# strawberrylady99/mythril

Measured on AMD Instinct MI355X. Metric: candidate assignments evaluated/sec (node) + time-to-first-model vs z3, higher is better.
Workload: dtype u32

## Files before the change

mythril_amd/csrc/jit_asm.cpp:

```cpp
#include <algorithm>
#include <array>
#include <cstdio>
#include <cstring>
#include <functional>
#include <map>
#include <set>
#include <sstream>
#include <string>
#include <vector>

#include "jit.hpp"

namespace mg {

namespace {

struct AsmFail {
  std::string why;
};
[[noreturn]] void fail(const std::string& w) { throw AsmFail{w}; }

inline uint32_t Lw(uint32_t w) { return (w + 31) / 32; }
inline uint32_t topmask(uint32_t w) { return (w & 31) ? ((1u << (w & 31)) - 1u) : 0xFFFFFFFFu; }
inline uint32_t gsalt(uint32_t c, uint32_t j) { return c * 0x9E3779B9u + j * 0x85EBCA6Bu + 0x27D4EB2Fu; }
// ... 241 lines not shown
    std::vector<int32_t> dix(P.vwidth.size(), -1);
    for (size_t k = 0; k < v.size(); k++)
      if (v[k].dst != MG_NONE && v[k].dst < dix.size() && dix[v[k].dst] < 0) dix[v[k].dst] = (int32_t)k;
    std::map<uint32_t, int32_t> coord_at;
    for (size_t k = 0; k < v.size(); k++)
      if (v[k].op == K_COORD && !coord_at.count(v[k].p0)) coord_at[v[k].p0] = (int32_t)k;
    auto operands = [&](const Instr& in, std::vector<int32_t>& out) {
      out.clear();
      auto add = [&](uint32_t id) {
        if (id != MG_NONE && id < dix.size() && dix[id] >= 0) out.push_back(dix[id]);
      };
      switch (in.op) {
        case K_CONST: break;
        case K_COORD:
          if (!eval_kernel && in.p0 < specs.size()) {
            const GenSpec& sp = specs[in.p0];
            if ((sp.kind & 0xFFu) == MG_GEN_MIXED && sp.p[3] != MG_NONE && (sp.p[2] & 0xFFFFu)) {
              auto it = coord_at.find(sp.p[3]);
              if (it != coord_at.end()) out.push_back(it->second);
            }
          }
          break;
        case K_LOOKUP:
          add(in.a);
          add(in.p0);
          for (uint32_t q = 0; q < 2 * in.c; q++) add(P.vaux[in.p1 + q]);
          break;
        case K_NOT: case K_NEG: case K_EXTRACT: case K_ZEXT: case K_SEXT: case K_ASSERT: case K_COPY: case K_WATCH:
          add(in.a);
          break;
        case K_ITE:
          add(in.a);
          add(in.b);
          add(in.c);
          break;
        default:
          add(in.a);
          add(in.b);
          break;
      }
    };
    std::vector<char> done(v.size(), 0);
    std::vector<Instr> out;
    out.reserve(v.size());
    std::vector<int32_t> ops;
    auto visit = [&](int32_t root) {
      std::vector<std::pair<int32_t, size_t>> st{{root, 0}};
      std::vector<std::vector<int32_t>> opl;
      opl.emplace_back();
      operands(v[root], opl.back());
      while (!st.empty()) {
        auto& top = st.back();
        if (done[top.first]) {
          st.pop_back();
          opl.pop_back();
          continue;
        }
        if (top.second < opl.back().size()) {
          const int32_t o = opl.back()[top.second++];
          if (!done[o]) {
            st.push_back({o, 0});
            opl.emplace_back();
            operands(v[o], opl.back());
          }
          continue;
        }
        done[top.first] = 1;
        out.push_back(v[top.first]);
        st.pop_back();
        opl.pop_back();
      }
    };
    if (eval_kernel && greedy_on()) {
      greedy_roots(v, operands, done, visit);
    } else if (!eval_kernel && heavy_last_on()) {
      heavy_last_roots(v, operands, done, visit);
    } else {
      for (size_t k = 0; k < v.size(); k++)
        if (v[k].op == K_ASSERT || v[k].op == K_WATCH) visit((int32_t)k);
    }
    for (size_t k = 0; k < v.size(); k++)
      if (!done[k]) visit((int32_t)k);
    code.swap(out);
  }
  static bool heavy_last_on() {
    static const bool on = [] {
      const char* g = getenv("MYTHGPU_JIT_ASM_HEAVY_LAST");
      return !(g && g[0] == '0');
    }();
    return on;
  }
  uint32_t op_weight(const Instr& in) const {
    const uint32_t w = (in.dst != MG_NONE && in.dst < P.vwidth.size()) ? P.vwidth[in.dst] : 32u;
    const uint32_t L = std::max(1u, Lw(std::max(w, in.op >= K_EQ && in.op <= K_UMUL_NOOVF ? in.p1 : w)));
    switch (in.op) {
      case K_KECCAK: return 2500u * (in.p0 / 136u + 1u);
      case K_EXP: return 1500u;
      case K_UDIV: case K_UREM: case K_SDIV: case K_SREM: case K_SMOD: return 600u;
      case K_MUL: return 4u * L * L;
      case K_UMUL_NOOVF: return 8u * L * L;
      case K_SHL: case K_LSHR: case K_ASHR: return 4u * L;
      case K_LOOKUP: return 2u * Lw(in.b) * std::max(1u, in.c);
      case K_COORD: return 8u * L;
      default: return L;
    }
  }
  static bool heavy_op(uint32_t op) {
    return op == K_KECCAK || op == K_EXP || op == K_UDIV || op == K_UREM || op == K_SDIV || op == K_SREM || op == K_SMOD;
  }
  template <class Ops, class Visit>
  void heavy_last_roots(const std::vector<Instr>& v, Ops& operands, const std::vector<char>& done, Visit& visit) {
    std::vector<int32_t> roots;
    for (size_t k = 0; k < v.size(); k++)
      if (v[k].op == K_ASSERT) roots.push_back((int32_t)k);
    std::vector<int32_t> mark(v.size(), -1), st, ops;
    int32_t stamp = 0;
    auto cone_cost = [&](int32_t r, bool& heavy) -> uint64_t {
      uint64_t c = 0;
      heavy = false;
      st.assign(1, r);
      mark[r] = ++stamp;
      while (!st.empty()) {
        const int32_t x = st.back();
        st.pop_back();
        c += op_weight(v[x]);
        heavy = heavy || heavy_op(v[x].op);
        operands(v[x], ops);
        for (int32_t o : ops)
          if (!done[o] && mark[o] != stamp) {
            mark[o] = stamp;
            st.push_back(o);
          }
      }
      return c;
    };
    std::vector<char> taken(roots.size(), 0);
    for (size_t step = 0; step < roots.size(); step++) {
      size_t pick = roots.size();
      uint64_t best = UINT64_MAX;
      for (size_t i = 0; i < roots.size(); i++) {
        if (taken[i]) continue;
        bool heavy = false;
        const uint64_t c = cone_cost(roots[i], heavy);
        if (!heavy) {
          pick = i;
          break;
        }
        if (c < best) {
          best = c;
          pick = i;
        }
      }
      taken[pick] = 1;
      visit(roots[pick]);
    }
  }
  static bool greedy_on() {
    static const bool on = [] {
      const char* g = getenv("MYTHGPU_JIT_ASM_GREEDY");
      return g && g[0] == '1';
    }();
    return on;
  }
  template <class Ops, class Visit>
  void greedy_roots(const std::vector<Instr>& v, Ops& operands, const std::vector<char>& done, Visit& visit) {
    const size_t n = v.size();
// ... 1108 lines not shown
    auto r = hby.equal_range(g);
    std::vector<std::vector<uint64_t>> keys;
    for (auto it = r.first; it != r.second; ++it) keys.push_back(it->second);
    hby.erase(r.first, r.second);
    for (const auto& k : keys) {
      auto it = hcache.find(k);
      if (it == hcache.end()) continue;
      const Limb d = it->second;
      hcache.erase(it);
      h_last.erase(k);
      drop(d);
    }
  }

  std::map<std::pair<uint32_t, uint32_t>, Limb> eqdiff;

  struct MEnt {
    Mask m;
    uint32_t tag = 0;
    uint64_t used = 0;
  };
  typedef std::vector<uint64_t> MKey;
  std::map<MKey, MEnt> mcache;
  uint32_t mc_hits = 0, mc_evictions = 0, mc_spills = 0;
  static bool no_mask_cache() {
    static const bool off = [] {
      const char* g = getenv("MYTHGPU_JIT_ASM_NO_MASK_CACHE");
      return g && g[0] == '1';
    }();
    return off;
  }
  bool mcache_on() const { return lvn_on && caches && !cond && !no_mask_cache(); }
  bool mcache_get(const MKey& key, Mask& m) {
    if (key.empty() || !mcache_on()) return false;
    auto it = mcache.find(key);
    if (it == mcache.end()) return false;
    E.scheck(it->second.m.s, it->second.tag);
    it->second.used = ++tick;
    m = it->second.m;
    E.sretain(m);
    mc_hits++;
    return true;
  }
  void mcache_put(const MKey& key, const Mask& m) {
    if (key.empty() || m.k != 2 || !mcache_on() || mcache.count(key)) return;
    MEnt e;
    e.m = m;
    e.tag = E.sgen[m.s];
    e.used = ++tick;
    E.sretain(m);
    mcache[key] = e;
  }
  bool mcache_evict() {
    auto best = mcache.end();
    for (auto it = mcache.begin(); it != mcache.end(); ++it)
      if (best == mcache.end() || it->second.used < best->second.used) best = it;
    if (best == mcache.end()) return false;
    E.srelease(best->second.m);
    mcache.erase(best);
    mc_evictions++;
    return true;
  }
  template <class F>
  void mcache_drop_if(F&& f) {
    for (auto it = mcache.begin(); it != mcache.end();) {
      if (f(it->first)) {
        E.srelease(it->second.m);
        it = mcache.erase(it);
      } else {
        ++it;
      }
    }
  }
  void mcache_forget(uint32_t id) {
    if (mcache.empty()) return;
    mcache_drop_if([&](const MKey& k) { return k[0] == 0 && (k[1] == id || k[2] == id); });
  }
  void mcache_free(uint32_t g) {
    if (mcache.empty()) return;
    mcache_drop_if([&](const MKey& k) { return (k[0] == 1 && k[1] == g) || (k[0] == 2 && (k[1] == g || k[3] == g)); });
  }
  void mcache_note() {
    E.o << "  ; mask cache: " << mc_hits << " hits, " << mc_evictions << " evictions, " << mc_spills << " mask spills\n";
  }
  int mcache_spare() const {
    int n = 0;
    for (const auto& kv : mcache) n += E.sref[kv.second.m.s] == 1;
    return n;
  }
  MKey idx_key(uint64_t kind, const Limb& idx) const {
    if (!idx.reg() || !idx.g || (int)idx.v < E.vfirst || E.vgen[idx.v] != idx.g) return {};
    return MKey{kind, idx.g, idx.v};
  }

  Mask eq_ids(uint32_t a, uint32_t b, uint32_t Lk) {
    PinScope pin_(*this, {a, b});
    const auto key = std::minmax(a, b);
    const MKey mkey{0, key.first, key.second};
    {
      Mask hit;
      if (mcache_get(mkey, hit)) {
        if (eqdiff.count(key)) eq_last[key] = ++tick;
        return hit;
      }
    }
    auto it = eqdiff.find(key);
    if (it != eqdiff.end()) {
      eq_last[key] = ++tick;
      Mask m;
      m.k = 2;
      m.s = E.salloc();
      E.valu("v_cmp_eq_u32_e64 " + SP(m.s) + ", 0, " + VL(it->second), {}, {m.s, m.s + 1});
      mcache_put(mkey, m);
      return m;
    }
    std::vector<std::pair<Limb, Limb>> prs;
    for (uint32_t j = 0; j < Lk; j++) prs.push_back({limb(a, j), limb(b, j)});
    Limb keep{};
    const Mask m = eq_mask(prs, &keep);
    if (keep.reg() && caches) {
      eqdiff[key] = keep;
      eq_last[key] = ++tick;
    }
    else if (keep.reg()) drop(keep);
    mcache_put(mkey, m);
    return m;
  }
  template <class M, class T>
  static typename M::iterator lru(M& m, T& last) {
    auto best = m.end();
    uint64_t bt = ~0ull;
    for (auto it = m.begin(); it != m.end(); ++it) {
      auto l = last.find(it->first);
      const uint64_t t = l == last.end() ? 0 : l->second;
      if (t < bt) {
        bt = t;
        best = it;
      }
    }
    return best;
  }
  bool evict_one() {
    if (!litcache.empty()) {
      auto it = lru(litcache, lit_last);
      const Limb d = it->second;
      lit_last.erase(it->first);
      litcache.erase(it);
      drop(d);
      return true;
    }
    if (!xcache.empty()) {
      auto it = lru(xcache, x_last);
      const Limb d = it->second;
      x_last.erase(it->first);
      xcache.erase(it);
      drop(d);
      return true;
    }
    if (!hcache.empty()) {
      auto it = lru(hcache, h_last);
      const Limb d = it->second;
      h_last.erase(it->first);
      hcache.erase(it);
      drop(d);
      return true;
    }
    if (!eqdiff.empty()) {
      auto it = lru(eqdiff, eq_last);
      const Limb d = it->second;
      eq_last.erase(it->first);
      eqdiff.erase(it);
      drop(d);
      return true;
    }
    return false;
  }
  size_t cur_k = 0;
  void note(const char* phase) {
    static const bool annotate = getenv("MYTHGPU_JIT_ASM_ANNOTATE") != nullptr;
    if (annotate) E.o << "  ; vcode " << cur_k << " " << phase << "\n";
  }
  bool spill_mask() {
    if (cond || cur_k >= code.size()) return false;
    const Instr& in = code[cur_k];
    auto operand = [&](uint32_t id) {
      if (id == in.a || id == in.b || id == in.c) return true;
      if (in.op == K_LOOKUP) {
        if (id == in.p0) return true;
        for (uint32_t q = 0; q < 2 * in.c; q++)
          if (P.vaux[in.p1 + q] == id) return true;
      }
      return false;
    };
    int64_t best = -1;
    int32_t bl = -1;
    for (uint32_t id = 0; id < val.size(); id++) {
      const Val& x = val[id];
      if (!x.def || x.m.k != 2 || E.sref[x.m.s] != 1 || operand(id)) continue;
      const int32_t lu = id < last.size() ? last[id] : -1;
      if (lu > bl) {
        bl = lu;
        best = id;
      }
// ... 1228 lines not shown
    if (!spill_on || cond) return false;
    int best = -1;
    int32_t bl = -1;
    for (uint32_t id = 0; id < val.size(); id++) {
      const Val& x = val[id];
      if (!x.def || is_spilled(id) || is_view(id) || P.vwidth[id] <= 32) continue;
      if (std::find(pinned.begin(), pinned.end(), id) != pinned.end()) continue;
      int regs = 0;
      bool own = true;
      for (const Limb& l : x.l)
        if (l.reg()) {
          regs++;
          own = own && (int)l.v >= E.vfirst && E.vref[l.v] == 1;
        }
      if (regs < 2 || !own) continue;
      const int32_t lu = id < last.size() ? last[id] : -1;
      if (lu > bl) {
        bl = lu;
        best = (int)id;
      }
    }
    if (best < 0) return false;
    Val& x = val[best];
    std::vector<int> at(x.l.size(), -1);
    for (size_t j = 0; j < x.l.size(); j++) {
      if (!x.l[j].reg()) continue;
      uint32_t sl = 0;
      while (sl < slot_busy.size() && slot_busy[sl]) sl++;
      if ((sl | 1u) > spill_cap()) fail("out of VGPRs (spill slots)");
      if (sl == slot_busy.size()) slot_busy.push_back(0);
      slot_busy[sl] = 1;
      spill_hwm = std::max(spill_hwm, sl + 1);
      E.mem("ds_write_b32 " + VL(spill_v) + ", " + VL(x.l[j]) + " offset:" + std::to_string(sl * 4u));
      at[j] = (int)sl;
    }
    E.ctl("s_waitcnt lgkmcnt(0)");
    for (size_t j = 0; j < x.l.size(); j++)
      if (at[j] >= 0) {
        drop(x.l[j]);
        x.l[j] = Limb{};
      }
    spill_at[best] = at;
    spills++;
    return true;
  }
  uint32_t spills = 0;
  void reload(uint32_t id) {
    if (cond) fail("a spilled value read under a branch");
    if (std::find(pinned.begin(), pinned.end(), id) == pinned.end())
      fail("internal: a spilled value read where it is not pinned");
    Val& x = val[id];
    const std::vector<int> at = spill_at[id];
    spill_at[id].clear();
    for (size_t j = 0; j < at.size(); j++) {
      if (at[j] < 0) continue;
      const Limb d = fresh();
      E.mem("ds_read_b32 " + VL(d) + ", " + VL(spill_v) + " offset:" + std::to_string((uint32_t)at[j] * 4u));
      x.l[j] = d;
    }
    E.ctl("s_waitcnt lgkmcnt(0)");
    for (int sl : at)
      if (sl >= 0) slot_busy[sl] = 0;
  }

  void kill(uint32_t id) {
    Val& x = val[id];
    if (is_spilled(id)) {
      for (int sl : spill_at[id])
        if (sl >= 0) slot_busy[sl] = 0;
      spill_at[id].clear();
    }
    for (auto& l : x.l) drop(l);
    x.l.clear();
    E.srelease(x.m);
    x.m = Mask{};
  }
  std::vector<Limb> limbs(uint32_t id, uint32_t n) {
    std::vector<Limb> r(n);
    for (uint32_t j = 0; j < n; j++) r[j] = limb(id, j);
    return r;
  }
  uint32_t demanded(uint32_t d) const { return need[d] ? 64 - (uint32_t)__builtin_clzll(need[d]) : 0; }

  bool lit_divisor(uint32_t b, uint32_t Ld) const {
    const Instr* bd = def_of(b);
    bool ok = bd && bd->op == K_CONST;
    for (uint32_t j = 1; ok && j < Ld; j++) ok = P.consts[bd->p0 + j] == 0;
    return ok;
  }
  void drop_all(std::vector<Limb>& v) {
    for (auto& x : v) drop(x);
    v.clear();
  }
  std::vector<Limb> own(const std::vector<Limb>& x, uint32_t n) {
    std::vector<Limb> r(n);
    for (uint32_t j = 0; j < n; j++) {
      const Limb s = j < x.size() && x[j].k != LU ? x[j] : Lit(0);
      r[j] = fresh();
      E.valu("v_mov_b32_e32 " + VL(r[j]) + ", " + src(s));
    }
    return r;
  }
  int sreg() { return E.salloc(); }
  void sfree(int s) {
    Mask m;
    m.k = 2;
    m.s = s;
    E.srelease(m);
  }
  Mask mask_new() {
    Mask m;
    m.k = 2;
    m.s = E.salloc();
    return m;
  }
  void vsel(const Limb& d, const Limb& f, const Limb& t, const Mask& m) {
    E.valu("v_cndmask_b32_e64 " + VL(d) + ", " + VL(f) + ", " + VL(t) + ", " + SP(m.s), {m.s, m.s + 1});
  }
  Mask vcmp(const char* op, const Limb& a, uint32_t k) {
    Mask m = mask_new();
    if (inl(k)) {
      E.valu(std::string("v_cmp_") + op + "_u32_e64 " + SP(m.s) + ", " + VL(a) + ", " + imm(k), {}, {m.s, m.s + 1});
    } else {
      E.salu("s_mov_b32 s41, " + hexs(k), {41});
      E.valu(std::string("v_cmp_") + op + "_u32_e64 " + SP(m.s) + ", " + VL(a) + ", s41", {41}, {m.s, m.s + 1});
    }
    return m;
  }

  Limb bitlen(const std::vector<Limb>& x) {
    const Limb bl = fresh();
    E.valu("v_mov_b32_e32 " + VL(bl) + ", 0");
    for (uint32_t j = 0; j < x.size(); j++) {
      const Limb l = x[j];
      if (l.k == LU || (l.lit() && l.v == 0)) continue;
      if (l.lit()) {
        E.valu("v_mov_b32_e32 " + VL(bl) + ", " + imm(32 * j + 32 - (uint32_t)__builtin_clz(l.v)));
        continue;
      }
      const Limb t = fresh();
      E.valu("v_ffbh_u32_e32 " + VL(t) + ", " + VL(l));
      E.valu("v_sub_u32_e32 " + VL(t) + ", " + imm(32 * j + 32) + ", " + VL(t));
      const Mask nz = vcmp("ne", l, 0);
      vsel(bl, bl, t, nz);
      E.srelease(nz);
      drop(t);
    }
    return bl;
  }
  void wave_max(const Limb& v, uint32_t bits, int s) {
    const int c = sreg();
    const Mask m = mask_new();
    E.salu("s_mov_b32 " + S(s) + ", 0", {s});
    for (int b = (int)bits - 1; b >= 0; b--) {
      E.salu("s_add_u32 " + S(c) + ", " + S(s) + ", " + imm(1u << b), {c});
      E.valu("v_cmp_ge_u32_e64 " + SP(m.s) + ", " + VL(v) + ", " + S(c), {c}, {m.s, m.s + 1});
      E.salu("s_cmp_lg_u64 " + SP(m.s) + ", 0");
      E.salu("s_cselect_b32 " + S(s) + ", " + S(c) + ", " + S(s), {s});
    }
    E.srelease(m);
    sfree(c);
  }

  void limb_barrel(std::vector<Limb>& x, const Limb& s, bool left, const Limb& fill) {
    const uint32_t Lx = (uint32_t)x.size();
    const Limb q = fresh();
// ... 1075 lines not shown
            r[j] = Lit(in.op == K_AND ? (a.v & b.v) : in.op == K_OR ? (a.v | b.v) : (a.v ^ b.v));
            continue;
          }
          const Limb l = a.lit() ? a : b, v = a.lit() ? b : a;
          if (l.lit()) {
            if ((in.op == K_AND && l.v == 0xFFFFFFFFu) || (in.op != K_AND && l.v == 0)) {
              E.retain(v);
              r[j] = v;
              continue;
            }
            if (in.op == K_AND && l.v == 0) { r[j] = Lit(0); continue; }
            if (in.op == K_OR && l.v == 0xFFFFFFFFu) { r[j] = Lit(0xFFFFFFFFu); continue; }
          }
          if (in.op != K_XOR && a == b) {
            E.retain(a);
            r[j] = a;
            continue;
          }
          const char* op = in.op == K_AND ? "v_and_b32_e32 " : in.op == K_OR ? "v_or_b32_e32 " : "v_xor_b32_e32 ";
          const Limb dd = fresh();
          E.valu(op + VL(dd) + ", " + src(l.lit() ? l : a) + ", " + VL(l.lit() ? v : b));
          r[j] = dd;
        }
        set(d, r);
        break;
      }
      case K_NOT: {
        if (W == 1) {
          set_mask(d, mnot(mask_of(in.a)));
          break;
        }
        std::vector<Limb> r(Ld);
        for (uint32_t j = 0; j < Ld; j++) {
          if (!(need[d] >> j & 1)) continue;
          const Limb a = limb(in.a, j);
          if (a.lit()) {
            r[j] = Lit(~a.v);
            continue;
          }
          const Limb dd = fresh();
          E.valu("v_not_b32_e32 " + VL(dd) + ", " + VL(a));
          r[j] = dd;
        }
        mask_top(r, W);
        set(d, r);
        break;
      }
      case K_COPY: {
        if (W == 1 && val[in.a].m.k) {
          E.sretain(val[in.a].m);
          val[d].m = val[in.a].m;
        }
        if (is_spilled(in.a)) reload(in.a);
        std::vector<Limb> r = val[in.a].l;
        for (auto& x : r) E.retain(x);
        set(d, r);
        break;
      }
      case K_ITE: {
        const Mask c = mask_of(in.a);
        if (W == 1) {
          if (c.k == 1) {
            const Mask x = mask_of(c.ones ? in.b : in.c);
            E.sretain(x);
            set_mask(d, x);
            break;
          }
          const Mask t = mop("and", c, mask_of(in.b));
          const Mask e = mask_of(in.c);
          Mask f;
          if (e.k == 1) {
            if (e.ones) {
              f = mnot(c);
            } else {
              f.k = 1;
              f.ones = false;
            }
          } else {
            f = mop_andn(e, c);
          }
          set_mask(d, mop("or", t, f));
          E.srelease(t);
          E.srelease(f);
          break;
        }
        std::vector<Limb> r(Ld);
        if (c.k == 1) {
          for (uint32_t j = 0; j < Ld; j++) {
            if (!(need[d] >> j & 1)) continue;
            r[j] = limb(c.ones ? in.b : in.c, j);
            E.retain(r[j]);
          }
          set(d, r);
          break;
        }
        if (c.k == 2 && !no_ite_e64() && !E.fresh_valu_write(c.s)) {
          for (uint32_t j = 0; j < Ld; j++) {
            if (!(need[d] >> j & 1)) continue;
            r[j] = sel_mask(limb(in.b, j), limb(in.c, j), c);
          }
          set(d, r);
          break;
        }
        mask_to_vcc(c);
        for (uint32_t j = 0; j < Ld; j++) {
          if (!(need[d] >> j & 1)) continue;
          r[j] = sel(limb(in.b, j), limb(in.c, j));
        }
        set(d, r);
        break;
      }
      case K_EQ: {
        const uint32_t La = Lw(in.p1);
        if (in.p1 == 1) {
          set_mask(d, mnot_xor(mask_of(in.a), mask_of(in.b)));
          break;
        }
        set_mask(d, no_eq_cache() ? [&] {
          std::vector<std::pair<Limb, Limb>> prs;
          for (uint32_t j = 0; j < La; j++) prs.push_back({limb(in.a, j), limb(in.b, j)});
          return eq_mask(prs);
        }() : eq_ids(in.a, in.b, La));
        break;
      }
      case K_ULT: case K_ULE: case K_SLT: case K_SLE: {
        const uint32_t La = Lw(in.p1);
        const bool sgn = in.op == K_SLT || in.op == K_SLE;
        if (in.p1 == 1) {
          const Mask a = mask_of(in.a), b = mask_of(in.b);
          Mask lt = sgn ? mop_andn(a, b) : mop_andn(b, a);
          if (in.op == K_ULE || in.op == K_SLE) {
            const Mask gt = sgn ? mop_andn(b, a) : mop_andn(a, b);
            const Mask le = mnot(gt);
            E.srelease(gt);
            E.srelease(lt);
            lt = le;
          }
          set_mask(d, lt);
          break;
        }
        slt_many = sgn && ((in.a < slt_lits.size() && slt_lits[in.a] >= 3) || (in.b < slt_lits.size() && slt_lits[in.b] >= 3));
        if (in.op == K_ULT || in.op == K_SLT) {
          set_mask(d, lt_mask(limbs(in.a, La), limbs(in.b, La), in.p1, sgn));
        } else {
          const Mask gt = lt_mask(limbs(in.b, La), limbs(in.a, La), in.p1, sgn);
          set_mask(d, mnot(gt));
          E.srelease(gt);
        }
        break;
      }
      case K_CONCAT: case K_EXTRACT: {
        std::vector<Limb> r(Ld);
        for (uint32_t j = 0; j < Ld; j++)
          if (need[d] >> j & 1) r[j] = field_of(in, 32 * j, std::min(32u, W - 32 * j));
        set(d, r);
        break;
      }
      case K_ZEXT: {
        const uint32_t La = Lw(in.p1);
        std::vector<Limb> r(Ld, Lit(0));
        for (uint32_t j = 0; j < La && j < Ld; j++) {
          if (!(need[d] >> j & 1)) continue;
          r[j] = limb(in.a, j);
          E.retain(r[j]);
        }
        set(d, r);
// ... 7 lines not shown
          r[j] = limb(in.a, j);
          E.retain(r[j]);
        }
        const Limb t = limb(in.a, La - 1);
        Limb top, f;
        if (t.lit()) {
          const uint32_t s = (wa - 1) & 31;
          const int32_t x = (int32_t)(t.v << (31 - s)) >> (31 - s);
          top = Lit((uint32_t)x);
          f = Lit(x < 0 ? 0xFFFFFFFFu : 0u);
        } else {
          if (wa & 31) {
            top = fresh();
            E.valu("v_bfe_i32 " + VL(top) + ", " + VL(t) + ", 0, " + std::to_string(wa & 31));
          } else {
            top = t;
            E.retain(top);
          }
          f = fresh();
          E.valu("v_ashrrev_i32_e32 " + VL(f) + ", 31, " + VL(top));
        }
        r[La - 1] = top;
        for (uint32_t j = La; j < Ld; j++) {
          r[j] = f;
          E.retain(f);
        }
        drop(f);
        mask_top(r, W);
        set(d, r);
        break;
      }
      case K_LOOKUP: {
        const uint32_t Lk = Lw(in.b), n = in.c;
        auto key_test = [&](uint32_t kv) -> Mask {
          if (!no_eq_cache()) return eq_ids(in.a, kv, Lk);
          std::vector<std::pair<Limb, Limb>> prs;
          for (uint32_t j = 0; j < Lk; j++) prs.push_back({limb(in.a, j), limb(kv, j)});
          return eq_mask(prs);
        };
        if (in.wd == 1 && !no_bool_lookup()) {
          Mask cur = mask_of(in.p0);
          E.sretain(cur);
          for (int32_t p = (int32_t)n - 1; p >= 0; p--) {
            const uint32_t kv = P.vaux[in.p1 + 2 * p], vv = P.vaux[in.p1 + 2 * p + 1];
            const Mask h = key_test(kv);
            if (h.k == 1) {
              if (h.ones) {
                E.srelease(cur);
                cur = mask_of(vv);
                E.sretain(cur);
              }
              continue;
            }
            const Mask vm = mask_of(vv);
            Mask nc;
            if (cur.k == 1 && !cur.ones) {
              nc = mop("and", h, vm);
            } else if (cur.k == 1 && vm.k == 2) {
              nc.k = 2;
              nc.s = E.salloc();
              E.salu("s_orn2_b64 " + SP(nc.s) + ", " + SP(vm.s) + ", " + SP(h.s), {nc.s, nc.s + 1});
            } else if (cur.k == 1) {
              if (vm.ones) {
                nc.k = 1;
                nc.ones = true;
              } else {
                nc = mnot(h);
              }
            } else if (vm.k == 1) {
              nc = vm.ones ? mop("or", h, cur) : mop_andn(cur, h);
            } else {
              const Mask t = mop("and", h, vm);
              const Mask f = mop_andn(cur, h);
              nc = mop("or", t, f);
              E.srelease(t);
              E.srelease(f);
            }
            E.srelease(cur);
            E.srelease(h);
            cur = nc;
          }
          set_mask(d, cur);
          break;
        }
        if (n >= 2 && n <= 5 && !no_lookup_runs() && E.sfree() + mcache_spare() >= (int)(n + n * (n - 1) / 2 + 4)) {
          std::vector<Mask> hs;
          std::vector<uint32_t> ps;
          int base = -1;
          for (int32_t p = (int32_t)n - 1; p >= 0; p--) {
            const Mask h = key_test(P.vaux[in.p1 + 2 * p]);
            if (h.k == 1) {
              if (h.ones) {
                for (auto& m : hs) E.srelease(m);
                hs.clear();
                ps.clear();
                base = p;
              }
              continue;
            }
            hs.push_back(h);
            ps.push_back((uint32_t)p);
          }
          const uint32_t dflt = base >= 0 ? P.vaux[in.p1 + 2 * base + 1] : in.p0;
          std::map<std::pair<size_t, size_t>, Mask> ors;
          auto run_mask = [&](size_t a, size_t b) -> Mask {
            if (a == b) return hs[a];
            auto it = ors.find({a, b});
            if (it != ors.end()) return it->second;
            const Mask prev = b - 1 == a ? hs[a] : ors.at({a, b - 1});
            const Mask m = mop("or", prev, hs[b]);
            ors[{a, b}] = m;
            return m;
          };
          std::vector<Limb> res(Ld);
          for (uint32_t j = 0; j < Ld; j++) {
            if (!(need[d] >> j & 1)) continue;
            Limb c = limb(dflt, j);
            E.retain(c);
            for (size_t a = 0; a < ps.size();) {
              const Limb v = limb(P.vaux[in.p1 + 2 * ps[a] + 1], j);
              size_t b = a;
              while (b + 1 < ps.size() && limb(P.vaux[in.p1 + 2 * ps[b + 1] + 1], j) == v) b++;
              if (!(v == c)) {
                for (size_t q = a + 1; q < b; q++) run_mask(a, q);
                const Mask m = run_mask(a, b);
                const Limb t = v3(v), f = v3(c);
                const Limb r = fresh();
                E.valu("v_cndmask_b32_e64 " + VL(r) + ", " + src(f) + ", " + src(t) + ", " + SP(m.s), {m.s, m.s + 1});
                drop(t);
                drop(f);
                drop(c);
                c = r;
              }
              a = b + 1;
            }
            res[j] = c;
          }
          for (auto& kv : ors) E.srelease(kv.second);
          for (auto& m : hs) E.srelease(m);
          set(d, res);
          break;
        }
        std::vector<Limb> cur(Ld);
        for (uint32_t j = 0; j < Ld; j++) {
          if (!(need[d] >> j & 1)) continue;
          cur[j] = limb(in.p0, j);
          E.retain(cur[j]);
        }
        for (int32_t p = (int32_t)n - 1; p >= 0; p--) {
          const uint32_t kv = P.vaux[in.p1 + 2 * p], vv = P.vaux[in.p1 + 2 * p + 1];
          Mask h;
          if (no_eq_cache()) {
            std::vector<std::pair<Limb, Limb>> prs;
            for (uint32_t j = 0; j < Lk; j++) prs.push_back({limb(in.a, j), limb(kv, j)});
            h = eq_mask(prs);
          } else {
            h = eq_ids(in.a, kv, Lk);
          }
          if (h.k == 1) {
            if (h.ones) {
              for (uint32_t j = 0; j < Ld; j++) {
                if (!(need[d] >> j & 1)) continue;
                drop(cur[j]);
                cur[j] = limb(vv, j);
                E.retain(cur[j]);
              }
// ... 92 lines not shown
    }();
    return on;
  }
  static bool no_bool_lookup() {
    static const bool on = [] {
      const char* g = getenv("MYTHGPU_JIT_ASM_NO_BOOL_LOOKUP");
      return g && g[0] == '1';
    }();
    return on;
  }
  static bool no_eq_cache() {
    static const bool on = [] {
      const char* g = getenv("MYTHGPU_JIT_ASM_NO_EQ_CACHE");
      return g && g[0] == '1';
    }();
    return on;
  }
  static bool gen_only() {
    static const bool on = [] {
      const char* g = getenv("MYTHGPU_JIT_ASM_GEN_ONLY");
      return g && g[0] == '1';
    }();
    return on;
  }
  static bool debug_live() {
    static const bool on = getenv("MYTHGPU_JIT_ASM_DEBUG") != nullptr;
    return on;
  }
  void operands_of(const Instr& in, size_t k, std::vector<uint32_t>& out) {
    std::function<void(uint32_t)> add = [&](uint32_t id) {
      if (id == MG_NONE || id >= val.size()) return;
      out.push_back(id);
      if (is_view(id)) {
        const Instr& vi = code[def[id]];
        add(vi.a);
        if (vi.op == K_CONCAT) add(vi.b);
      }
    };
    switch (in.op) {
      case K_CONST: break;
      case K_COORD: if (copysrc[k] != MG_NONE) add(copysrc[k]); break;
      case K_LOOKUP:
        add(in.a);
        add(in.p0);
        for (uint32_t q = 0; q < in.c; q++) add(P.vaux[in.p1 + 2 * q + 1]);
        break;
      default:
        add(in.a);
        if (in.op != K_NOT && in.op != K_NEG && in.op != K_EXTRACT && in.op != K_ZEXT && in.op != K_SEXT &&
            in.op != K_ASSERT && in.op != K_COPY && in.op != K_WATCH)
          add(in.b);
        if (in.op == K_ITE) add(in.c);
        break;
    }
  }
  void body(const std::string& next) {
    eqdiff.clear();
    mcache.clear();
    mc_hits = mc_evictions = mc_spills = 0;
    mulshare.clear();
    xcache.clear();
    xby.clear();
    hcache.clear();
    hby.clear();
    h_last.clear();
    litcache.clear();
    lit_last.clear();
    x_last.clear();
    eq_last.clear();
    dlimb.clear();
    E.on_free = [this](uint32_t g) {
      xcache_free(g);
      hcache_free(g);
      dlimb_free(g);
      mcache_free(g);
    };
    E.on_pressure = [this]() { return evict_one(); };
    E.on_hard = [this]() { return spill_one(); };
    spill_at.assign(val.size(), {});
    slot_busy.clear();
    pinned.clear();
    E.on_spressure = [this]() { return mcache_evict() || spill_mask(); };
    lvn_on = true;
    static const bool annotate = getenv("MYTHGPU_JIT_ASM_ANNOTATE") != nullptr;
    for (size_t k = 0; k < code.size(); k++) {
      const Instr& in = code[k];
      cur_k = k;
      if (is_view(in.dst)) continue;
      if (annotate)
        E.o << "  ; vcode " << k << " op " << in.op << " w " << in.wd << " dst " << in.dst << " a " << in.a << " b " << in.b
            << "\n";
      if (spill_on) {
        pinned.clear();
        operands_of(in, k, pinned);
        for (size_t q = 0; q < pinned.size(); q++)
          if (is_spilled(pinned[q])) reload(pinned[q]);
      }
      emit(in, k, next);
      if (spill_on) pinned.clear();
      if (debug_live()) {
        int used = 0;
        for (int r = E.vfirst; r < 256; r++) used += E.vref[r] > 0;
        fprintf(stderr, "asm live %zu op %u w %u: %d VGPRs\n", k, in.op, in.wd, used);
        static const long at = getenv("MYTHGPU_JIT_ASM_DEBUG_AT") ? atol(getenv("MYTHGPU_JIT_ASM_DEBUG_AT")) : -1;
        if ((long)k == at) {
          std::map<uint32_t, int> byop;
          for (uint32_t id = 0; id < val.size(); id++) {
            if (!val[id].def) continue;
            int regs = 0;
            for (const auto& l : val[id].l) regs += l.reg();
            if (regs && def[id] >= 0) byop[code[def[id]].op] += regs;
          }
          for (const auto& kv : byop) fprintf(stderr, "  live from op %u: %d limbs\n", kv.first, kv.second);
        }
      }
      auto done = [&](uint32_t id) {
        if (id != MG_NONE && id < last.size() && last[id] <= (int32_t)k && val[id].def) {
          kill(id);
          val[id].def = false;
          if (!eqdiff.empty()) eq_forget(id);
          mcache_forget(id);
        }
      };
      if (in.dst != MG_NONE && in.dst < last.size() && last[in.dst] < 0) done(in.dst);
      switch (in.op) {
        case K_CONST: break;
        case K_WATCH:
          if (eval_kernel) done(in.a);
          break;
        case K_COORD:
          if (copysrc[k] != MG_NONE) done(copysrc[k]);
          break;
        case K_LOOKUP:
          done(in.a);
          done(in.p0);
          for (uint32_t q = 0; q < 2 * in.c; q++) done(P.vaux[in.p1 + q]);
          break;
        default:
          done(in.a);
          if (in.b != MG_NONE) done(in.b);
          if (in.op == K_ITE) done(in.c);
          if (in.op == K_CONCAT || in.op == K_EXTRACT) {
            std::function<void(uint32_t)> through = [&](uint32_t id) {
              if (!is_view(id)) return;
              const Instr& vi = code[def[id]];
              done(vi.a);
              through(vi.a);
              if (vi.op == K_CONCAT) {
                done(vi.b);
                through(vi.b);
              }
            };
            through(in.a);
            if (in.op == K_CONCAT) through(in.b);
          }
          break;
      }
    }
    for (auto& kv : mulshare)
      for (auto& t : kv.second) drop(t);
    mulshare.clear();
    for (auto& kv : eqdiff) drop(kv.second);
    eqdiff.clear();
    mcache_drop_if([](const MKey&) { return true; });
    xcache_clear();
    litcache_clear();
    lvn_on = false;
    E.on_free = nullptr;
    E.on_pressure = nullptr;
    E.on_hard = nullptr;
// ... 711 lines not shown
      << "    .amdhsa_user_sgpr_count 2\n    .amdhsa_user_sgpr_kernarg_segment_ptr 1\n"
      << "    .amdhsa_system_sgpr_workgroup_id_x 1\n    .amdhsa_system_vgpr_workitem_id 0\n"
      << "    .amdhsa_next_free_vgpr " << nv << "\n    .amdhsa_next_free_sgpr " << ns << "\n"
      << "    .amdhsa_accum_offset " << accum << "\n    .amdhsa_reserve_vcc 1\n"
      << "    .amdhsa_float_denorm_mode_32 3\n    .amdhsa_float_denorm_mode_16_64 3\n"
      << "  .end_amdhsa_kernel\n  .text\n";
    labels = E.nlab;
    meta_lds = lds_words * 4;
    meta_vgpr[name] = nv;
    meta_sgpr[name] = ns + 6;
    return o.str();
  }
  std::map<std::string, int> meta_vgpr, meta_sgpr;
  uint32_t meta_lds = 0;
};

std::string metadata(const std::map<std::string, int>& vg, const std::map<std::string, int>& sg, bool with_gen,
                     uint32_t lds_bytes) {
  std::ostringstream o;
  auto arg = [&](uint32_t off, uint32_t size, const char* kind, bool global) {
    o << "      - .offset: " << off << "\n        .size: " << size << "\n        .value_kind: " << kind << "\n";
    if (global) o << "        .address_space: global\n";
  };
  o << "  .amdgpu_metadata\n---\namdhsa.kernels:\n";
  for (const char* name : {"mgj_search", "mgj_gen"}) {
    const bool gen = std::strcmp(name, "mgj_gen") == 0;
    if (gen && !with_gen) continue;
    o << "  - .args:\n";
    arg(0, 8, "global_buffer", true);
    for (uint32_t k = 0; k < 4; k++) arg(8 + 8 * k, 8, "by_value", false);
    arg(40, 8, "global_buffer", true);
    if (gen) {
      arg(48, 4, "by_value", false);
    } else {
      arg(48, 4, "by_value", false);
      arg(52, 4, "by_value", false);
    }
    o << "    .group_segment_fixed_size: " << lds_bytes << "\n    .kernarg_segment_align: 8\n"
      << "    .kernarg_segment_size: " << (gen ? 52 : 56) << "\n    .max_flat_workgroup_size: 256\n"
      << "    .name: " << name << "\n    .private_segment_fixed_size: 0\n"
      << "    .sgpr_count: " << sg.at(name) << "\n    .sgpr_spill_count: 0\n"
      << "    .symbol: " << name << ".kd\n    .uniform_work_group_size: 1\n    .uses_dynamic_stack: false\n"
      << "    .vgpr_count: " << vg.at(name) << "\n    .vgpr_spill_count: 0\n    .wavefront_size: 64\n"
      << "    .agpr_count: 0\n";
  }
  o << "amdhsa.target: amdgcn-amd-amdhsa--gfx950\namdhsa.version:\n  - 1\n  - 2\n...\n  .end_amdgpu_metadata\n";
  return o.str();
}

}

std::string metadata_eval(int vg, int sg, uint32_t lds) {
  std::ostringstream o;
  auto arg = [&](uint32_t off, uint32_t size, const char* kind, bool global) {
    o << "      - .offset: " << off << "\n        .size: " << size << "\n        .value_kind: " << kind << "\n";
    if (global) o << "        .address_space: global\n";
  };
  o << "  .amdgpu_metadata\n---\namdhsa.kernels:\n  - .args:\n";
  arg(0, 8, "global_buffer", true);
  arg(8, 8, "by_value", false);
  arg(16, 8, "global_buffer", true);
  arg(24, 8, "global_buffer", true);
  arg(32, 4, "by_value", false);
  o << "    .group_segment_fixed_size: " << lds << "\n    .kernarg_segment_align: 8\n    .kernarg_segment_size: 36\n"
    << "    .max_flat_workgroup_size: 256\n    .name: mgj_eval\n    .private_segment_fixed_size: 0\n"
    << "    .sgpr_count: " << sg << "\n    .sgpr_spill_count: 0\n    .symbol: mgj_eval.kd\n"
    << "    .uniform_work_group_size: 1\n    .uses_dynamic_stack: false\n    .vgpr_count: " << vg
    << "\n    .vgpr_spill_count: 0\n    .wavefront_size: 64\n    .agpr_count: 0\n"
    << "amdhsa.target: amdgcn-amd-amdhsa--gfx950\namdhsa.version:\n  - 1\n  - 2\n...\n  .end_amdgpu_metadata\n";
  return o.str();
}

constexpr double kSgkeyRatio = 0.25;

static int occupancy_step(int v) {
  static const int floor_v = [] {
    const char* g = getenv("MYTHGPU_JIT_ASM_VMIN");
    return g ? std::max(24, std::min(256, atoi(g))) : 96;
  }();
  const int waves = std::max(1, std::min(8, 512 / ((std::max(v, 1) + 7) / 8 * 8)));
  return std::max(floor_v, std::min(256, 512 / waves / 8 * 8));
}

int jit_asm_source(const Lowered& P, const std::vector<GenSpec>& specs, const std::vector<uint32_t>& gconsts,
                   uint32_t kernels, std::string& out, std::string& err) {
  try {
    Gen g(P, specs, gconsts);
    std::ostringstream o;
    o << kAsmMarker << "\n  .amdgcn_target \"amdgcn-amd-amdhsa--gfx950\"\n  .amdhsa_code_object_version 6\n";
    if (kernels & JIT_EVAL) try {
      if (const char* st = getenv("MYTHGPU_JIT_ASM_SPILL_TEST")) throw AsmFail{"out of VGPRs (spill test " + std::string(st) + ")"};
      g.eval_kernel = true;
      g.tiled = (kernels & JIT_EVAL_TILED) || getenv("MYTHGPU_JIT_ASM_TILED");
      g.analyse();
      g.depth = Gen::prefetch_env() ? Gen::prefetch_env() : 8u;
      g.caches = false;
      std::string ks;
      int nv;
      try {
        ks = g.kernel_eval("mgj_eval");
        nv = g.meta_vgpr["mgj_eval"];
      } catch (const AsmFail&) {
        nv = 256;
      }
      const int waves = std::max(1, std::min(8, 512 / ((nv + 7) / 8 * 8)));
      const int budget = std::min(256, 512 / waves / 8 * 8);
      g.caches = true;
      g.vsoft = budget;
      g.labels = 0;
      ks = g.kernel_eval("mgj_eval");
      if (!Gen::prefetch_env()) {
        for (int d = std::min(60, 8 + budget - nv); d > 8; d -= 4) {
          g.depth = (uint32_t)d;
          g.labels = 0;
          try {
            std::string k2 = g.kernel_eval("mgj_eval");
            if (g.meta_vgpr["mgj_eval"] <= budget) {
              ks = k2;
              break;
            }
          } catch (const AsmFail&) {
            g.meta_vgpr["mgj_eval"] = 1 << 20;
          }
        }
        if (g.meta_vgpr["mgj_eval"] > budget) {
          g.depth = 8;
          g.labels = 0;
          ks = g.kernel_eval("mgj_eval");
        }
      }
      if (g.tiled && Gen::glds_env()) {
        const std::string vks = ks;
        const uint32_t vdepth = g.depth;
        const int vnv = g.meta_vgpr["mgj_eval"];
        const uint32_t M = (uint32_t)g.rows.size();
        auto depth_for = [&](int nv) {
          if (Gen::glds_fixed()) return std::min<uint32_t>(Gen::glds_fixed(), M);
          const int w = std::max(1, std::min(8, 512 / ((nv + 7) / 8 * 8)));
          const int slots = 160 / w;
          return std::min<uint32_t>({32u, M, (uint32_t)std::max(1, (slots - 1) / 2)});
        };
        g.gdepth = depth_for(vnv);
        bool ok = true;
        try {
          g.labels = 0;
          ks = g.kernel_eval("mgj_eval");
          const uint32_t d2 = depth_for(g.meta_vgpr["mgj_eval"]);
          if (d2 != g.gdepth) {
            g.gdepth = d2;
            g.labels = 0;
            ks = g.kernel_eval("mgj_eval");
          }
        } catch (const AsmFail&) {
          ok = false;
        }
        if (!ok || (!Gen::glds_fixed() && g.gdepth <= vdepth)) {
          g.gdepth = 0;
          g.depth = vdepth;
          g.glds = false;
          ks = vks;
          g.meta_vgpr["mgj_eval"] = vnv;
        }
      }
      if (!getenv("MYTHGPU_JIT_ASM_NOPOOL")) {
        std::vector<std::pair<uint32_t, uint32_t>> by;
        for (const auto& kv : g.census)
          if (kv.second >= 2) by.push_back({kv.second, kv.first});
        std::sort(by.begin(), by.end(), [](const auto& a, const auto& b) { return a.first > b.first; });
        const int room = std::max(0, 96 - g.meta_vgpr["mgj_eval"]);
        for (size_t i = 0; i < by.size() && (int)i < room; i++) g.pool[by[i].second] = kV0 + (int)i;
        if (!g.pool.empty()) {
          g.labels = 0;
          ks = g.kernel_eval("mgj_eval");
        }
      }
      o << ks << metadata_eval(g.meta_vgpr["mgj_eval"], g.meta_sgpr["mgj_eval"], g.eval_lds_bytes());
      out = o.str();
      return MG_OK;
    } catch (const AsmFail& f) {
      const char* ns = getenv("MYTHGPU_JIT_ASM_NO_SPILL");
      if ((ns && ns[0] == '1') || f.why.find("out of VGPRs") == std::string::npos) throw;
      Gen g2(P, specs, gconsts);
      g2.eval_kernel = true;
      g2.tiled = (kernels & JIT_EVAL_TILED) || getenv("MYTHGPU_JIT_ASM_TILED");
      g2.analyse();
      g2.spill_on = true;
      g2.depth = 8;
      g2.gdepth = 0;
      g2.caches = true;
      g2.vsoft = 256;
      if (const char* st = getenv("MYTHGPU_JIT_ASM_SPILL_TEST")) g2.vhard = g2.vsoft = std::max(24, std::min(256, atoi(st)));
      g2.labels = 0;
      std::string ks;
      try {
        ks = g2.kernel_eval("mgj_eval");
      } catch (const AsmFail& f2) {
        if (f2.why.find("spill slots") == std::string::npos) throw;
        g2.solo = true;
        g2.labels = 0;
        ks = g2.kernel_eval("mgj_eval");
      }
      o << ks << metadata_eval(g2.meta_vgpr["mgj_eval"], g2.meta_sgpr["mgj_eval"], g2.eval_lds_bytes());
      out = o.str();
      return MG_OK;
    }
    g.analyse();
    g.gen_kernel = false;
    g.caches = false;
    std::string ks;
    int v0;
    try {
      ks = g.kernel("mgj_search");
      v0 = g.meta_vgpr["mgj_search"];
      if (getenv("MYTHGPU_JIT_ASM_VREPORT")) fprintf(stderr, "mythgpu asm: pass-1 VGPRs %d\n", v0);
    } catch (const AsmFail&) {
      v0 = 256;
      g.census.clear();
    }
    g.caches = true;
    g.vsoft = occupancy_step(v0);
    if (Gen::sgkey_env() >= 0) {
      g.sgkey = Gen::sgkey_env() == 1;
    } else if (!ks.empty()) {
      size_t sa = 0, va = 0;
      std::istringstream in(ks);
      for (std::string ln; std::getline(in, ln);) {
        if (ln.rfind("  v_", 0) == 0) va++;
        else if (ln.rfind("  s_", 0) == 0 && ln.rfind("  s_waitcnt", 0) && ln.rfind("  s_nop", 0) &&
                 ln.rfind("  s_branch", 0) && ln.rfind("  s_cbranch", 0) && ln.rfind("  s_endpgm", 0))
          sa++;
      }
      g.sgkey = va && (double)sa < kSgkeyRatio * (double)va;
    }
    {
      std::vector<std::pair<uint32_t, uint32_t>> by;
      static const uint32_t pool_min = [] {
        const char* g = getenv("MYTHGPU_JIT_ASM_POOL_MIN");
        return g ? (uint32_t)std::max(1, atoi(g)) : 2u;
      }();
      if (!getenv("MYTHGPU_JIT_ASM_NOPOOL"))
        for (const auto& kv : g.census)
          if (kv.second >= pool_min) by.push_back({kv.second, kv.first});
      std::sort(by.begin(), by.end(), [](const auto& a, const auto& b) { return a.first > b.first; });
      const int room = std::max(0, std::min(96, g.vsoft) - v0);
      for (size_t i = 0; i < by.size() && (int)i < room; i++) g.pool[by[i].second] = kV0 + (int)i;
      g.labels = 0;
      ks = g.kernel("mgj_search");
    }
    o << ks;
    const bool with_gen = (kernels & JIT_GEN) != 0;
    if (with_gen) {
      g.gen_kernel = true;
      o << g.kernel("mgj_gen");
    }
    o << metadata(g.meta_vgpr, g.meta_sgpr, with_gen, g.meta_lds);
    out = o.str();
    return MG_OK;
  } catch (const AsmFail& f) {
    err = f.why;
    return MG_E_UNSUPPORTED;
  } catch (const std::exception& x) {
    err = std::string("assembly tier: ") + x.what();
    return MG_E_UNSUPPORTED;
  }
}

}
```

Baseline: 280.7 billion.

## Guard heavy ITE arms and lookup runs behind wave-uniform branches in search kernel

Adds a planning pass that sinks the single-use cone of instructions feeding one ITE arm right before the ITE, then at codegen wraps that region in an s_cbranch that skips it when the condition mask is uniformly against that arm for the whole wavefront. Small lookup runs get the same treatment, skipping the select chain when no lane matches a key. The aim is to avoid evaluating dead arms per wave, paid for with extra scalar branches, region copies and invalidation of cached boolean state. Generation falls back to a non-lazy kernel if the lazy build fails, and it caps the VGPR budget at 64 when guards exist.

```diff
diff --git a/mythril_amd/csrc/jit_asm.cpp b/mythril_amd/csrc/jit_asm.cpp
--- a/mythril_amd/csrc/jit_asm.cpp
+++ b/mythril_amd/csrc/jit_asm.cpp
@@ -347,6 +347,163 @@
     for (size_t k = 0; k < v.size(); k++)
       if (!done[k]) visit((int32_t)k);
     code.swap(out);
+    guards.clear();
+    if (lazy && !eval_kernel) plan_lazy();
+  }
+
+  bool lazy = true;
+  static bool no_lazy() {
+    static const bool on = [] {
+      const char* g = getenv("MYTHGPU_JIT_ASM_NO_LAZY");
+      return g && g[0] == '1';
+    }();
+    return on;
+  }
+  static uint32_t lazy_min() {
+    static const uint32_t n = [] {
+      const char* g = getenv("MYTHGPU_JIT_ASM_LAZY_MIN");
+      return g ? (uint32_t)std::max(0, atoi(g)) : 8u;
+    }();
+    return n;
+  }
+  static uint32_t lazy_priors() {
+    static const uint32_t n = [] {
+      const char* g = getenv("MYTHGPU_JIT_ASM_LAZY_PRIORS");
+      return g ? (uint32_t)std::max(0, std::min(8, atoi(g))) : 1u;
+    }();
+    return n;
+  }
+  struct Guard {
+    uint32_t dst = MG_NONE;
+    uint32_t size = 0;
+    bool true_arm = true;
+    uint32_t weight = 0;
+    int32_t ite = -1, begin = -1;
+  };
+  std::vector<Guard> guards;
+  std::vector<int32_t> guard_of;
+  std::vector<std::vector<int32_t>> guard_begin;
+  template <class F>
+  void reads(const Instr& in, F&& f) const {
+    auto r = [&](uint32_t id) {
+      if (id != MG_NONE && id < P.vwidth.size()) f(id);
+    };
+    switch (in.op) {
+      case K_CONST: case K_COORD: break;
+      case K_LOOKUP:
+        r(in.a);
+        r(in.p0);
+        for (uint32_t q = 0; q < 2 * in.c; q++) r(P.vaux[in.p1 + q]);
+        break;
+      case K_NOT: case K_NEG: case K_EXTRACT: case K_ZEXT: case K_SEXT: case K_ASSERT: case K_COPY: case K_WATCH:
+        r(in.a);
+        break;
+      case K_ITE:
+        r(in.a);
+        r(in.b);
+        r(in.c);
+        break;
+      default:
+        r(in.a);
+        r(in.b);
+        break;
+    }
+  }
+  void plan_lazy() {
+    const size_t nv = P.vwidth.size(), n = code.size();
+    std::vector<char> fixed_coord(specs.size(), 0);
+    {
+      std::vector<uint32_t> times(specs.size(), 0);
+      for (const GenSpec& sp : specs)
+        if ((sp.kind & 0xFFu) == MG_GEN_MIXED && sp.p[3] != MG_NONE && sp.p[3] < specs.size()) fixed_coord[sp.p[3]] = 1;
+      for (const Instr& in : code)
+        if (in.op == K_COORD && in.p0 < specs.size() && ++times[in.p0] > 1) fixed_coord[in.p0] = 1;
+    }
+    std::vector<uint32_t> defs(nv, 0);
+    for (const Instr& in : code)
+      if (in.dst != MG_NONE && in.dst < nv) defs[in.dst]++;
+    std::vector<std::vector<int32_t>> users(nv);
+    auto index_users = [&]() {
+      for (auto& u : users) u.clear();
+      for (size_t p = 0; p < n; p++) reads(code[p], [&](uint32_t id) { users[id].push_back((int32_t)p); });
+    };
+    index_users();
+    std::vector<char> in_cone(n, 0);
+    auto cone_of = [&](int32_t K, uint32_t arm, std::vector<int32_t>& cone, uint32_t& weight) {
+      cone.clear();
+      weight = 0;
+      for (int32_t p = K - 1; p >= 0; p--) {
+        in_cone[p] = 0;
+        const Instr& in = code[p];
+        const uint32_t d = in.dst;
+        if (d == MG_NONE || d >= nv || defs[d] != 1 || users[d].empty() || heavy_op(in.op)) continue;
+        if (in.op == K_COORD && (in.p0 >= specs.size() || fixed_coord[in.p0])) continue;
+        bool all = true;
+        for (int32_t u : users[d]) all = all && (u == K ? d == arm : (u < K && in_cone[u]));
+        if (!all) continue;
+        in_cone[p] = 1;
+        cone.push_back(p);
+        if (in.op != K_CONST) weight += op_weight(in);
+      }
+      std::reverse(cone.begin(), cone.end());
+    };
+    std::vector<int32_t> cone, cone2;
+    std::vector<Instr> moved;
+    for (int32_t K = 0; K < (int32_t)n; K++) {
+      const Instr in = code[K];
+      if (in.op != K_ITE || in.dst == MG_NONE || in.dst >= nv || P.vwidth[in.dst] <= 1 || defs[in.dst] != 1) continue;
+      if (in.a == in.b || in.a == in.c || in.b == in.c || in.a >= nv || in.b >= nv || in.c >= nv) continue;
+      const uint32_t Ld = L(in.dst);
+      bool taken = false;
+      for (int t = 0; t < 2 && !taken; t++) {
+        const bool true_arm = t == 0;
+        const uint32_t arm = true_arm ? in.b : in.c, other = true_arm ? in.c : in.b;
+        uint32_t weight = 0;
+        cone_of(K, arm, cone, weight);
+        if (cone.empty()) continue;
+        bool dies = true;
+        for (int32_t u : users[other]) dies = dies && u <= K;
+        const uint32_t copies = dies ? 0u : Ld;
+        if (!true_arm && copies) continue;
+        if (weight + Ld < lazy_min() + copies) continue;
+        const int32_t lo = cone.front();
+        moved.clear();
+        for (int32_t p = lo; p < K; p++)
+          if (!in_cone[p]) moved.push_back(code[p]);
+        for (int32_t p : cone) moved.push_back(code[p]);
+        std::copy(moved.begin(), moved.end(), code.begin() + lo);
+        Guard g;
+        g.dst = in.dst;
+        g.size = (uint32_t)cone.size();
+        g.true_arm = true_arm;
+        g.weight = weight;
+        guards.push_back(g);
+        index_users();
+        taken = true;
+      }
+    }
+    std::vector<int32_t> at(nv, -1);
+    for (size_t p = 0; p < n; p++)
+      if (code[p].dst != MG_NONE && code[p].dst < nv && at[code[p].dst] < 0) at[code[p].dst] = (int32_t)p;
+    guard_of.assign(n, -1);
+    guard_begin.assign(n, {});
+    std::vector<Guard> kept;
+    for (Guard g : guards) {
+      g.ite = at[g.dst];
+      g.begin = g.ite - (int32_t)g.size;
+      const Instr& in = code[g.ite];
+      const uint32_t other = g.true_arm ? in.c : in.b;
+      if (g.begin < 0 || at[in.a] >= g.begin || at[other] >= g.begin) continue;
+      kept.push_back(g);
+    }
+    guards.swap(kept);
+    std::vector<int32_t> order(guards.size());
+    for (size_t i = 0; i < order.size(); i++) order[i] = (int32_t)i;
+    std::sort(order.begin(), order.end(), [&](int32_t x, int32_t y) { return guards[x].ite > guards[y].ite; });
+    for (int32_t i : order) {
+      guard_of[guards[i].ite] = i;
+      guard_begin[guards[i].begin].push_back(i);
+    }
   }
   static bool heavy_last_on() {
     static const bool on = [] {
@@ -1621,6 +1778,7 @@
   }
   void mcache_note() {
     E.o << "  ; mask cache: " << mc_hits << " hits, " << mc_evictions << " evictions, " << mc_spills << " mask spills\n";
+    if (lazy && !eval_kernel) E.o << "  ; lazy arms: " << lazy_regions << " guarded regions\n";
   }
   int mcache_spare() const {
     int n = 0;
@@ -1657,7 +1815,7 @@
     for (uint32_t j = 0; j < Lk; j++) prs.push_back({limb(a, j), limb(b, j)});
     Limb keep{};
     const Mask m = eq_mask(prs, &keep);
-    if (keep.reg() && caches) {
+    if (keep.reg() && caches && !cond) {
       eqdiff[key] = keep;
       eq_last[key] = ++tick;
     }
@@ -3052,6 +3210,105 @@
   }
   uint32_t demanded(uint32_t d) const { return need[d] ? 64 - (uint32_t)__builtin_clzll(need[d]) : 0; }
 
+  struct Region {
+    bool active = false;
+    Mask c;
+    bool true_arm = true;
+    std::vector<Limb> r;
+    std::string skip;
+    std::vector<std::pair<uint32_t, uint8_t>> bools;
+  };
+  std::vector<Region> regions;
+  uint32_t lazy_regions = 0;
+  bool in_place(const Limb& x, uint32_t u, size_t k) const {
+    return x.reg() && (int)x.v >= E.vfirst && E.vref[x.v] == 1 && last[u] <= (int32_t)k;
+  }
+  uint32_t region_copies(uint32_t u, uint32_t d, size_t k) {
+    uint32_t n = 0;
+    for (uint32_t j = 0; j < L(d); j++)
+      if (need[d] >> j & 1) n += !in_place(limb(u, j), u, k);
+    return n;
+  }
+  void region_open(Region& rg, const Mask& c, bool true_arm, uint32_t u, uint32_t d, size_t k) {
+    rg = Region{};
+    rg.active = true;
+    rg.c = c;
+    rg.true_arm = true_arm;
+    E.sretain(c);
+    const uint32_t Ld = L(d);
+    rg.r.assign(Ld, Limb{});
+    for (uint32_t j = 0; j < Ld; j++) {
+      if (!(need[d] >> j & 1)) continue;
+      const Limb x = limb(u, j);
+      if (in_place(x, u, k)) {
+        E.retain(x);
+        rg.r[j] = x;
+      } else {
+        const Limb f = fresh();
+        E.valu("v_mov_b32_e32 " + VL(f) + ", " + src(x));
+        rg.r[j] = f;
+      }
+    }
+    for (uint32_t id = 0; id < val.size(); id++) {
+      const Val& x = val[id];
+      if (!x.def || P.vwidth[id] != 1) continue;
+      rg.bools.push_back({id, (uint8_t)((x.m.k ? 1 : 0) | ((!x.l.empty() && x.l[0].k != LU) ? 2 : 0))});
+    }
+    rg.skip = E.newlab();
+    cond++;
+    lazy_regions++;
+    note(true_arm ? "lazy:guard" : "lazy:guard-else");
+    E.salu("s_cmp_eq_u64 " + SP(c.s) + ", " + (true_arm ? "0" : "-1"));
+    E.ctl("s_cbranch_scc1 " + rg.skip);
+    note("lazy:region");
+  }
+  void region_select(Region& rg, uint32_t arm, const Mask* by = nullptr) {
+    {
+      size_t n = 0;
+      for (const Limb& l : rg.r) n += l.k != LU;
+      note(("lazy:select x" + std::to_string(n)).c_str());
+    }
+    const Mask& m = by ? *by : rg.c;
+    for (uint32_t j = 0; j < rg.r.size(); j++) {
+      if (rg.r[j].k == LU) continue;
+      const Limb a = v3(limb(arm, j));
+      const std::string f = rg.true_arm ? VL(rg.r[j]) : src(a), t = rg.true_arm ? src(a) : VL(rg.r[j]);
+      E.valu("v_cndmask_b32_e64 " + VL(rg.r[j]) + ", " + f + ", " + t + ", " + SP(m.s), {m.s, m.s + 1});
+      drop(a);
+    }
+  }
+  void region_close(Region& rg, uint32_t d) {
+    E.label(rg.skip);
+    cond--;
+    for (const auto& b : rg.bools) {
+      Val& x = val[b.first];
+      if (!x.def) continue;
+      if (!(b.second & 1) && x.m.k) {
+        E.srelease(x.m);
+        x.m = Mask{};
+      }
+      if (!(b.second & 2) && !x.l.empty()) {
+        for (auto& l : x.l) drop(l);
+        x.l.clear();
+      }
+    }
+    E.srelease(rg.c);
+    rg.active = false;
+    set(d, rg.r);
+  }
+  void guard_open(int32_t gi) {
+    const Guard& gd = guards[gi];
+    const Instr& in = code[gd.ite];
+    Region& rg = regions[gi];
+    rg = Region{};
+    if (!cond) sreserve();
+    const Mask c = mask_of(in.a);
+    if (c.k != 2) return;
+    const uint32_t u = gd.true_arm ? in.c : in.b, copies = region_copies(u, in.dst, (size_t)gd.ite);
+    if ((!gd.true_arm && copies) || gd.weight + L(in.dst) < lazy_min() + copies) return;
+    region_open(rg, c, gd.true_arm, gd.true_arm ? in.c : in.b, in.dst, (size_t)gd.ite);
+  }
+
   bool lit_divisor(uint32_t b, uint32_t Ld) const {
     const Instr* bd = def_of(b);
     bool ok = bd && bd->op == K_CONST;
@@ -4293,6 +4550,12 @@
           set_mask(d, mop("or", t, f));
           E.srelease(t);
           E.srelease(f);
+          break;
+        }
+        if (!guards.empty() && guard_of[k] >= 0 && regions[guard_of[k]].active) {
+          Region& rg = regions[guard_of[k]];
+          region_select(rg, rg.true_arm ? in.b : in.c);
+          region_close(rg, d);
           break;
         }
         std::vector<Limb> r(Ld);
@@ -4466,6 +4729,34 @@
           }
           set_mask(d, cur);
           break;
+        }
+        if (lazy && !eval_kernel && n >= 1 && n <= lazy_priors() && last[in.p0] <= (int32_t)k &&
+            (uint32_t)__builtin_popcountll(need[d] & lowmask(Ld)) * n >=
+                std::max(1u, lazy_min()) + region_copies(in.p0, d, k)) {
+          if (!cond) sreserve();
+          std::vector<Mask> hs(n);
+          bool pairs = true;
+          for (uint32_t p = 0; p < n; p++) {
+            hs[p] = key_test(P.vaux[in.p1 + 2 * p]);
+            pairs = pairs && hs[p].k == 2;
+          }
+          if (pairs) {
+            Mask any = hs[0];
+            E.sretain(any);
+            for (uint32_t p = 1; p < n; p++) {
+              const Mask o = mop("or", any, hs[p]);
+              E.srelease(any);
+              any = o;
+            }
+            Region rg;
+            region_open(rg, any, true, in.p0, d, k);
+            E.srelease(any);
+            for (int32_t p = (int32_t)n - 1; p >= 0; p--) region_select(rg, P.vaux[in.p1 + 2 * p + 1], &hs[p]);
+            for (auto& h : hs) E.srelease(h);
+            region_close(rg, d);
+            break;
+          }
+          for (auto& h : hs) E.srelease(h);
         }
         if (n >= 2 && n <= 5 && !no_lookup_runs() && E.sfree() + mcache_spare() >= (int)(n + n * (n - 1) / 2 + 4)) {
           std::vector<Mask> hs;
@@ -4724,10 +5015,15 @@
     pinned.clear();
     E.on_spressure = [this]() { return mcache_evict() || spill_mask(); };
     lvn_on = true;
+    cond = 0;
+    regions.assign(guards.size(), Region{});
+    lazy_regions = 0;
     static const bool annotate = getenv("MYTHGPU_JIT_ASM_ANNOTATE") != nullptr;
     for (size_t k = 0; k < code.size(); k++) {
       const Instr& in = code[k];
       cur_k = k;
+      if (!guards.empty())
+        for (int32_t gi : guard_begin[k]) guard_open(gi);
       if (is_view(in.dst)) continue;
       if (annotate)
         E.o << "  ; vcode " << k << " op " << in.op << " w " << in.wd << " dst " << in.dst << " a " << in.a << " b " << in.b
@@ -5605,6 +5901,8 @@
   return std::max(floor_v, std::min(256, 512 / waves / 8 * 8));
 }
 
+static std::string search_kernels(Gen& g, uint32_t kernels, bool strict);
+
 int jit_asm_source(const Lowered& P, const std::vector<GenSpec>& specs, const std::vector<uint32_t>& gconsts,
                    uint32_t kernels, std::string& out, std::string& err) {
   try {
@@ -5727,6 +6025,35 @@
       out = o.str();
       return MG_OK;
     }
+    g.lazy = !Gen::no_lazy();
+    if (g.lazy) {
+      std::string o2;
+      try {
+        o2 = search_kernels(g, kernels, true);
+      } catch (const AsmFail&) {
+        o2.clear();
+      }
+      if (!o2.empty()) {
+        out = o.str() + o2;
+        return MG_OK;
+      }
+    }
+    Gen g0(P, specs, gconsts);
+    g0.lazy = false;
+    out = o.str() + search_kernels(g0, kernels, false);
+    return MG_OK;
+  } catch (const AsmFail& f) {
+    err = f.why;
+    return MG_E_UNSUPPORTED;
+  } catch (const std::exception& x) {
+    err = std::string("assembly tier: ") + x.what();
+    return MG_E_UNSUPPORTED;
+  }
+}
+
+static std::string search_kernels(Gen& g, uint32_t kernels, bool strict) {
+  std::ostringstream o;
+  {
     g.analyse();
     g.gen_kernel = false;
     g.caches = false;
@@ -5737,11 +6064,13 @@
       v0 = g.meta_vgpr["mgj_search"];
       if (getenv("MYTHGPU_JIT_ASM_VREPORT")) fprintf(stderr, "mythgpu asm: pass-1 VGPRs %d\n", v0);
     } catch (const AsmFail&) {
+      if (strict) throw;
       v0 = 256;
       g.census.clear();
     }
     g.caches = true;
     g.vsoft = occupancy_step(v0);
+    if (g.lazy && !g.guards.empty() && v0 <= 64) g.vsoft = 64;
     if (Gen::sgkey_env() >= 0) {
       g.sgkey = Gen::sgkey_env() == 1;
     } else if (!ks.empty()) {
@@ -5777,15 +6106,8 @@
       o << g.kernel("mgj_gen");
     }
     o << metadata(g.meta_vgpr, g.meta_sgpr, with_gen, g.meta_lds);
-    out = o.str();
-    return MG_OK;
-  } catch (const AsmFail& f) {
-    err = f.why;
-    return MG_E_UNSUPPORTED;
-  } catch (const std::exception& x) {
-    err = std::string("assembly tier: ") + x.what();
-    return MG_E_UNSUPPORTED;
-  }
+  }
+  return o.str();
 }
 
 }
```

New measurement: 324.2 billion, median of 6. +15.5%, better.
